# yjpark1/multiagent_rl

Measured on NVIDIA B200. Metric: agent-steps/sec, higher is better.
Workload: dtype f32

## Files before the change

multiagent_rl_b200/csrc/actor_launch.h:

```cpp
#pragma once
#include <cuda_runtime.h>
#include <stdint.h>

#include "env_launch.h"

namespace mpe {

constexpr int kActorMaxD = 64;
constexpr int kActorMaxA = 16;
constexpr int kHid = 64;
constexpr int kH = 32;
constexpr int kGateK = 96;
constexpr int kGateN = 128;

struct TcDev {
  unsigned char *blob = nullptr;
  uint32_t bytes = 0;
  int D = 0, Kx = 0, A0 = 0, A1 = 0, A = 0;
  uint32_t off_wih[2][2] = {}, off_whh[2][2] = {}, off_w1[2] = {};
  uint32_t off_w2f = 0, off_bg = 0, off_b1 = 0, off_b2 = 0;
  float *scratch = nullptr;
};

enum { kImplAuto = 0, kImplSimt = 1, kImplTc = 2, kImplTcFusedLarge = 3 };

struct ActorDev {
  TcDev tc;
  int impl = kImplAuto;
  float *blob = nullptr;
  size_t blob_floats = 0;
  size_t smem_floats = 0;
  int D = 0, A0 = 0, A1 = 0, A = 0, Apad = 0, Dpad = 0, has_model = 0;
  int off_wg[2] = {0, 0};
  int off_bg = 0;
  int off_w1 = 0;
  int off_b1 = 0;
  int off_w2 = 0;
  int off_b2 = 0;
  int off_w3 = 0;
  int off_b3 = 0;
};

struct ActorHostWeights {
  const float *dense1_w, *dense1_b, *w_ih, *w_hh, *b_ih, *b_hh, *w_ih_r, *w_hh_r, *b_ih_r, *b_hh_r;
  const float *dense2_w, *dense2_b, *dense2b_w, *dense2b_b, *dense3_w, *dense3_b;
};

struct ActorIO {
  const float *obs = nullptr;
  const float *gumbel = nullptr;
  float *logits = nullptr;
  float *next_state = nullptr;
  int32_t *act_u = nullptr, *act_c = nullptr;
  float *onehot = nullptr;
  float *hcat = nullptr;
  int64_t B = 0, gid0 = 0;
  int32_t N = 0;
  uint64_t seed = 0, step = 0;
};

struct RolloutIO {
  int32_t T = 0;
  uint64_t step0 = 0;
  float *obs_next = nullptr;
  float *rew = nullptr;
  int32_t *act_u = nullptr, *act_c = nullptr;
  float *obs_work = nullptr;
};

void actor_layout(int D, int A0, int A1, bool has_model, ActorDev *out);
void actor_pack(const ActorDev &d, const ActorHostWeights &w, float *host_blob);
bool actor_supported(int N);
bool rollout_supported(int scenario, int N);
// ... 13 lines not shown
```

multiagent_rl_b200/csrc/common.cuh:

```cuda
#pragma once
#include <cuda_runtime.h>
#include <stdint.h>

namespace mpe {

constexpr int kWarp = 32;

enum : uint32_t { kDomainReset = 1, kDomainGoal = 2, kDomainGumbel = 3, kDomainRespawn = 4 };

__device__ __forceinline__ uint4 philox4x32_10(uint4 c, uint2 k) {
#pragma unroll
  for (int r = 0; r < 10; ++r) {
    const uint32_t hi0 = __umulhi(0xD2511F53u, c.x), lo0 = 0xD2511F53u * c.x;
    const uint32_t hi1 = __umulhi(0xCD9E8D57u, c.z), lo1 = 0xCD9E8D57u * c.z;
    c = make_uint4(hi1 ^ c.y ^ k.x, lo1, hi0 ^ c.w ^ k.y, lo0);
    k.x += 0x9E3779B9u;
    k.y += 0xBB67AE85u;
  }
  return c;
}

__device__ __forceinline__ uint4 philox_raw(uint64_t seed, uint64_t gid, uint32_t t, uint32_t domain,
                                            uint32_t slot) {
  return philox4x32_10(make_uint4((uint32_t)gid, (uint32_t)(gid >> 32), t, (domain << 16) | slot),
// ... 102 lines not shown
}

__device__ __forceinline__ uint32_t smem_u32(const void *p) {
  return (uint32_t)__cvta_generic_to_shared(p);
}

__device__ __forceinline__ void fence_proxy_async_smem() {
  asm volatile("fence.proxy.async.shared::cta;" ::: "memory");
}

__device__ __forceinline__ void bulk_store(void *gdst, const void *ssrc, uint32_t bytes) {
  asm volatile("cp.async.bulk.global.shared::cta.bulk_group [%0], [%1], %2;" ::"l"(gdst),
               "r"(smem_u32(ssrc)), "r"(bytes)
               : "memory");
}
__device__ __forceinline__ void bulk_commit() { asm volatile("cp.async.bulk.commit_group;" ::: "memory"); }
__device__ __forceinline__ void bulk_wait_read_all() {
  asm volatile("cp.async.bulk.wait_group.read 0;" ::: "memory");
}
__device__ __forceinline__ void bulk_wait_read_1() {
  asm volatile("cp.async.bulk.wait_group.read 1;" ::: "memory");
}

__device__ __forceinline__ void mbar_init(uint64_t *bar, uint32_t count) {
  asm volatile("mbarrier.init.shared::cta.b64 [%0], %1;" ::"r"(smem_u32(bar)), "r"(count) : "memory");
}
__device__ __forceinline__ void mbar_fence_init() {
  asm volatile("fence.mbarrier_init.release.cluster;" ::: "memory");
}
__device__ __forceinline__ void mbar_expect_tx(uint64_t *bar, uint32_t bytes) {
  asm volatile("mbarrier.arrive.expect_tx.shared::cta.b64 _, [%0], %1;" ::"r"(smem_u32(bar)), "r"(bytes)
               : "memory");
}
__device__ __forceinline__ void mbar_wait(uint64_t *bar, uint32_t parity) {
  asm volatile(
      "{\n\t"
      ".reg .pred p;\n\t"
      "WAIT_%=:\n\t"
      "mbarrier.try_wait.parity.shared::cta.b64 p, [%0], %1, %2;\n\t"
      "@p bra DONE_%=;\n\t"
      "bra WAIT_%=;\n\t"
      "DONE_%=:\n\t"
      "}" ::"r"(smem_u32(bar)),
      "r"(parity), "r"(1000000u)
      : "memory");
}
__device__ __forceinline__ void bulk_load(void *sdst, const void *gsrc, uint32_t bytes, uint64_t *bar) {
  asm volatile(
      "cp.async.bulk.shared::cluster.global.mbarrier::complete_tx::bytes [%0], [%1], %2, [%3];" ::"r"(
          smem_u32(sdst)),
      "l"(gsrc), "r"(bytes), "r"(smem_u32(bar))
      : "memory");
}

}
```

multiagent_rl_b200/csrc/env_core.cuh:

```cuda
#pragma once
#include <cmath>
#include <type_traits>

#include "common.cuh"

namespace mpe {

enum : int { kSpread = 0, kReference = 1, kSpeaker = 2, kTreasure = 3 };

template <int SC, int N_>
struct Dims {
  static constexpr int N = N_;
  static constexpr int L = (SC == kSpread) ? N_ : 3;
  static constexpr int D = (SC == kSpread) ? 4 + 2 * L : (SC == kReference ? 21 : 11);
  static constexpr int DIMC = (SC == kSpread) ? 2 : (SC == kReference ? 10 : 3);
  static constexpr int R = N * D;
  static constexpr bool kCollide = (SC == kSpread);
  static constexpr bool kHasGoal = (SC != kSpread);
  static constexpr bool kTalks = (SC == kReference);
};

template <typename T>
struct EnvState {
  T *pv;
// ... 133 lines not shown
__device__ __forceinline__ T mul_rn(T a, T b) { return a * b; }
template <>
__device__ __forceinline__ float mul_rn<float>(float a, float b) { return __fmul_rn(a, b); }

template <typename T>
__device__ __forceinline__ void integrate_agent(T &px, T &py, T &vx, T &vy, T fx, T fy, T max_speed) {
  T vxi = mad<T>(fx, (T)0.1, mul_rn<T>(vx, (T)0.75));
  T vyi = mad<T>(fy, (T)0.1, mul_rn<T>(vy, (T)0.75));
  if (max_speed >= (T)0) {
    const T speed = sqrt(sq2<T>(vxi, vyi));
    if (speed > max_speed) {
      vxi = vxi / speed * max_speed;
      vyi = vyi / speed * max_speed;
    }
  }
  vx = vxi; vy = vyi;
  px = mad<T>(vxi, (T)0.1, px);
  py = mad<T>(vyi, (T)0.1, py);
}

template <typename T, int SC, int N>
struct Env {
  using Dm = Dims<SC, N>;
  static constexpr int L = Dm::L;
  static constexpr int D = Dm::D;
  T px[N], py[N], vx[N], vy[N];
  T lx[L], ly[L];
  int goal[2];

  __device__ __forceinline__ static T size_of_agent() {
    return SC == kSpread ? (T)0.15 : (SC == kReference ? (T)0.05 : (T)0.075);
  }
  __device__ __forceinline__ static bool movable(int i) { return !(SC == kSpeaker && i == 0); }

  __device__ __forceinline__ void load(const EnvState<T> &s, int64_t b) {
#pragma unroll
    for (int i = 0; i < N; ++i) {
      const Vec4<T> v = ld4(s.pv + ((int64_t)i * s.B + b) * 4);
      px[i] = v.x; py[i] = v.y; vx[i] = v.z; vy[i] = v.w;
    }
#pragma unroll
    for (int l = 0; l < L; ++l) {
      const Vec2<T> v = ld2(s.lm + ((int64_t)l * s.B + b) * 2);
      lx[l] = v.x; ly[l] = v.y;
    }
    goal[0] = goal[1] = -1;
    if (Dm::kHasGoal) {
      const int32_t g = s.goal[b];
      goal[0] = (g & 0xFF) == 0xFF ? -1 : (g & 0xFF);
      goal[1] = ((g >> 8) & 0xFF) == 0xFF ? -1 : ((g >> 8) & 0xFF);
    }
  }

  __device__ __forceinline__ void store_agents(const EnvState<T> &s, int64_t b) const {
#pragma unroll
    for (int i = 0; i < N; ++i) st4(s.pv + ((int64_t)i * s.B + b) * 4, Vec4<T>{px[i], py[i], vx[i], vy[i]});
  }
  __device__ __forceinline__ void store_world(const EnvState<T> &s, int64_t b) const {
#pragma unroll
    for (int l = 0; l < L; ++l) st2(s.lm + ((int64_t)l * s.B + b) * 2, Vec2<T>{lx[l], ly[l]});
    if (Dm::kHasGoal) s.goal[b] = (goal[0] & 0xFF) | ((goal[1] & 0xFF) << 8);
  }

  __device__ __forceinline__ void reset(uint64_t seed, uint64_t gid, uint32_t episode) {
    constexpr int E = N + L;
#pragma unroll
    for (int j = 0; j < (E + 1) / 2; ++j) {
      const uint4 r = philox_raw(seed, gid, episode, kDomainReset, j);
      set_entity_pos(2 * j, bits_to_pos<T>(r.x), bits_to_pos<T>(r.y));
      if (2 * j + 1 < E) set_entity_pos(2 * j + 1, bits_to_pos<T>(r.z), bits_to_pos<T>(r.w));
    }
#pragma unroll
    for (int i = 0; i < N; ++i) vx[i] = vy[i] = (T)0;
    goal[0] = goal[1] = -1;
    if (Dm::kHasGoal) {
      const uint4 r = philox_raw(seed, gid, episode, kDomainGoal, 0);
      goal[0] = (int)__umulhi(r.x, (uint32_t)L);
      if (SC == kReference) goal[1] = (int)__umulhi(r.y, (uint32_t)L);
    }
  }
  __device__ __forceinline__ void set_entity_pos(int e, T x, T y) {
    if (e < N) { px[e] = x; py[e] = y; }
    else { lx[e - N] = x; ly[e - N] = y; }
  }

  __device__ __forceinline__ void physics(const int *act_u, const EnvState<T> &s) {
    const T max_speed = s.max_speed;
    const T sens = s.accel >= (T)0 ? s.accel : (T)5.0;
    T fx[N], fy[N];
#pragma unroll
    for (int i = 0; i < N; ++i) {
      const int a = act_u[i];
      const T u0 = (T)0 + ((a == 1 ? (T)1 : (T)0) - (a == 2 ? (T)1 : (T)0));
      const T u1 = (T)0 + ((a == 3 ? (T)1 : (T)0) - (a == 4 ? (T)1 : (T)0));
      fx[i] = u0 * sens;
      fy[i] = u1 * sens;
    }
    if (Dm::kCollide) {
      const T dist_min = size_of_agent() + size_of_agent();
#pragma unroll
      for (int a = 0; a < N; ++a) {
#pragma unroll
        for (int b = a + 1; b < N; ++b) {
          const T dx = px[a] - px[b], dy = py[a] - py[b];
          const T d2 = sq2<T>(dx, dy);
          if (std::is_same<T, float>::value || !(d2 >= s.t2_cut)) {
// ... 114 lines not shown
```

multiagent_rl_b200/csrc/tc_kernels.cu:

```cuda
#include <cuda_fp16.h>

#include <cstdlib>
#include <cstring>

#include "actor_launch.h"
#include "env_core.cuh"
#include "env_group.cuh"
#include "tc_common.cuh"

namespace mpe {

constexpr int kTcThreads = 320;
constexpr int kRows = 128;
constexpr float kWScale = 16.0f, kWInv = 0.0625f, kLog2e = 1.4426950408889634f;
constexpr uint32_t kChunkA = kRows * 16;

void tc_layout(int D, int A0, int A1, TcDev *o) {
  o->D = D; o->A0 = A0; o->A1 = A1; o->A = A0 + A1;
  o->Kx = D <= 16 ? 16 : (D <= 32 ? 32 : 0);
  uint32_t off = 0;
  for (int d = 0; d < 2; ++d)
    for (int hl = 0; hl < 2; ++hl) { o->off_wih[d][hl] = off; off += kHid * kGateN * 2; }
  for (int d = 0; d < 2; ++d)
    for (int hl = 0; hl < 2; ++hl) { o->off_whh[d][hl] = off; off += kH * kGateN * 2; }
  for (int hl = 0; hl < 2; ++hl) { o->off_w1[hl] = off; off += (o->Kx > 0 ? o->Kx : 16) * kHid * 2; }
  o->off_w2f = off; off += kHid * 16 * 4;
  o->off_bg = off; off += 2 * kGateN * 4;
  o->off_b1 = off; off += kHid * 4;
  o->off_b2 = off; off += 16 * 4;
  o->bytes = (off + 127) / 128 * 128;
}

bool tc_supported(const TcDev &t) { return t.Kx > 0 && t.A <= 16; }

static void put_split(unsigned char *img, uint32_t off_hi, uint32_t off_lo, int rows, int n, int k, float v) {
  const float x = v * kWScale;
  const __half hi = __float2half_rn(x);
  const __half lo = __float2half_rn(x - __half2float(hi));
  const size_t idx = ((size_t)(k / 8) * rows + n) * 8 + (k % 8);
  reinterpret_cast<__half *>(img + off_hi)[idx] = hi;
  reinterpret_cast<__half *>(img + off_lo)[idx] = lo;
}

void tc_pack(const TcDev &t, const ActorHostWeights &w, unsigned char *img) {
  std::memset(img, 0, t.bytes);
  const float *wih[2] = {w.w_ih, w.w_ih_r}, *whh[2] = {w.w_hh, w.w_hh_r};
  const float *bih[2] = {w.b_ih, w.b_ih_r}, *bhh[2] = {w.b_hh, w.b_hh_r};
  float *bg = reinterpret_cast<float *>(img + t.off_bg);
  for (int d = 0; d < 2; ++d)
    for (int g = 0; g < 4; ++g)
      for (int u = 0; u < kH; ++u) {
        const int row = g * kH + u, n = (u >> 1) * 8 + g * 2 + (u & 1);
        for (int k = 0; k < kHid; ++k) put_split(img, t.off_wih[d][0], t.off_wih[d][1], kGateN, n, k, wih[d][row * kHid + k]);
        for (int k = 0; k < kH; ++k) put_split(img, t.off_whh[d][0], t.off_whh[d][1], kGateN, n, k, whh[d][row * kH + k]);
        bg[d * kGateN + n] = (bih[d][row] + bhh[d][row]) * (g == 2 ? -2.0f : -1.0f) * kLog2e;
      }
  float *b1 = reinterpret_cast<float *>(img + t.off_b1), *b2 = reinterpret_cast<float *>(img + t.off_b2);
  for (int j = 0; j < kHid; ++j) {
    for (int k = 0; k < t.D; ++k) put_split(img, t.off_w1[0], t.off_w1[1], kHid, j, k, w.dense1_w[j * t.D + k]);
    b1[j] = w.dense1_b[j];
  }
  for (int a = 0; a < t.A; ++a) {
    const float *src = a < t.A0 ? w.dense2_w + a * kHid : w.dense2b_w + (a - t.A0) * kHid;
    for (int k = 0; k < kHid; ++k) reinterpret_cast<float *>(img + t.off_w2f)[k * 16 + a] = src[k];
    b2[a] = a < t.A0 ? w.dense2_b[a] : w.dense2b_b[a - t.A0];
  }
}


__device__ __forceinline__ void mbar_arrive(uint64_t *bar) {
  asm volatile("mbarrier.arrive.shared::cta.b64 _, [%0];" ::"r"(smem_u32(bar)) : "memory");
}
__device__ __forceinline__ void bar_sync_n(int id, int n) { asm volatile("bar.sync %0, %1;" ::"r"(id), "r"(n) : "memory"); }

__device__ __forceinline__ void store_chunk_split(unsigned char *hi_chunk, unsigned char *lo_chunk, int row,
                                                  const float (&v)[8]) {
  uint32_t h[4], l[4];
#pragma unroll
  for (int i = 0; i < 4; ++i) {
    __half h0, l0, h1, l1;
    split_f16(v[2 * i], h0, l0);
    split_f16(v[2 * i + 1], h1, l1);
    h[i] = pack_h2(h0, h1);
    l[i] = pack_h2(l0, l1);
  }
  *reinterpret_cast<uint4 *>(hi_chunk + row * 16) = make_uint4(h[0], h[1], h[2], h[3]);
  *reinterpret_cast<uint4 *>(lo_chunk + row * 16) = make_uint4(l[0], l[1], l[2], l[3]);
}

__device__ __forceinline__ void mma3_ss(uint32_t tmem_d, const unsigned char *a_hi, const unsigned char *a_lo,
                                        uint32_t a_lbo, const unsigned char *b_hi, const unsigned char *b_lo,
                                        uint32_t b_lbo, int kblocks, uint32_t idesc, bool accumulate) {
  for (int kb = 0; kb < kblocks; ++kb) {
    const uint64_t ah = make_smem_desc(a_hi + kb * 2 * a_lbo, a_lbo, 128), al = make_smem_desc(a_lo + kb * 2 * a_lbo, a_lbo, 128);
    const uint64_t bh = make_smem_desc(b_hi + kb * 2 * b_lbo, b_lbo, 128), bl = make_smem_desc(b_lo + kb * 2 * b_lbo, b_lbo, 128);
    mma_f16_ss(tmem_d, ah, bh, idesc, accumulate || kb > 0);
    mma_f16_ss(tmem_d, al, bh, idesc, true);
    mma_f16_ss(tmem_d, ah, bl, idesc, true);
  }
}
__device__ __forceinline__ void mma3_ts(uint32_t tmem_d, uint32_t a_hi, uint32_t a_lo, const unsigned char *b_hi,
                                        const unsigned char *b_lo, uint32_t b_lbo, int kblocks, uint32_t idesc,
                                        bool accumulate) {
  for (int kb = 0; kb < kblocks; ++kb) {
    const uint64_t bh = make_smem_desc(b_hi + kb * 2 * b_lbo, b_lbo, 128), bl = make_smem_desc(b_lo + kb * 2 * b_lbo, b_lbo, 128);
    mma_f16_ts(tmem_d, a_hi + kb * 8, bh, idesc, accumulate || kb > 0);
    mma_f16_ts(tmem_d, a_lo + kb * 8, bh, idesc, true);
    mma_f16_ts(tmem_d, a_hi + kb * 8, bl, idesc, true);
  }
}

__device__ unsigned long long g_tc_timeline[148 * 128];
#ifdef MPE_TC_PHASES
#define TL(role, i)                                                                                              \
  do {                                                                                                           \
    if (dbg && first_tile && blockIdx.x < 148) g_tc_timeline[blockIdx.x * 128 + (role) * 32 + (i)] = clock64(); \
  } while (0)
#else
#define TL(role, i)
#endif

enum { B_X = 0, B_D1, B_H1, B_G, B_H, B_PER_WG };

__host__ __device__ constexpr int tc_x_slots(int N) { return N <= 3 ? N : (N <= 6 ? 4 : 2); }
__host__ __device__ inline size_t tc_x_bytes(int N, int Kx) { return (size_t)tc_x_slots(N) * 2 * (Kx / 8) * kChunkA; }
__host__ __device__ inline size_t tc_smem_bytes(uint32_t wbytes, int N, int Kx) {
  return (size_t)wbytes + 2 * (tc_x_bytes(N, Kx) + 16384 + (size_t)((kRows * N * 2 + 127) / 128 * 128)) + (1 + 2 * B_PER_WG) * 8 + 64;
}

__device__ __forceinline__ float ex2_approx(float x) {
  float y;
  asm("ex2.approx.ftz.f32 %0, %1;" : "=f"(y) : "f"(x));
  return y;
}
__device__ __forceinline__ float exp_neg(float x) { return ex2_approx(fminf(-1.4426950408889634f * x, 57.0f)); }

__device__ __forceinline__ void dense1_half(const uint32_t (&v)[32], const float *b1, uint32_t taddr_hi,
                                            uint32_t lo_off = 32) {
  uint32_t hi[16], lo[16];
#pragma unroll
  for (int j = 0; j < 16; ++j) {
    const float2 bj = *reinterpret_cast<const float2 *>(b1 + 2 * j);
    const float a0 = fmaxf(fmaf(__uint_as_float(v[2 * j]), kWInv, bj.x), 0.0f);
    const float a1 = fmaxf(fmaf(__uint_as_float(v[2 * j + 1]), kWInv, bj.y), 0.0f);
    __half h0, l0, h1, l1;
    split_f16(a0, h0, l0);
    split_f16(a1, h1, l1);
    hi[j] = pack_h2(h0, h1);
    lo[j] = pack_h2(l0, l1);
  }
  tmem_st16(taddr_hi, hi);
  tmem_st16(taddr_hi + lo_off, lo);
}

typedef unsigned long long f2;
__device__ __forceinline__ f2 pk(float lo, float hi) { f2 r; asm("mov.b64 %0, {%1, %2};" : "=l"(r) : "f"(lo), "f"(hi)); return r; }
__device__ __forceinline__ f2 pk(uint32_t lo, uint32_t hi) { f2 r; asm("mov.b64 %0, {%1, %2};" : "=l"(r) : "r"(lo), "r"(hi)); return r; }
__device__ __forceinline__ void upk(f2 v, float &lo, float &hi) { asm("mov.b64 {%0, %1}, %2;" : "=f"(lo), "=f"(hi) : "l"(v)); }
__device__ __forceinline__ f2 fma2(f2 a, f2 b, f2 c) { f2 d; asm("fma.rn.f32x2 %0, %1, %2, %3;" : "=l"(d) : "l"(a), "l"(b), "l"(c)); return d; }
__device__ __forceinline__ f2 add2(f2 a, f2 b) { f2 d; asm("add.rn.f32x2 %0, %1, %2;" : "=l"(d) : "l"(a), "l"(b)); return d; }
__device__ __forceinline__ f2 mul2(f2 a, f2 b) { f2 d; asm("mul.rn.f32x2 %0, %1, %2;" : "=l"(d) : "l"(a), "l"(b)); return d; }
__device__ __forceinline__ float rcp_approx(float x) { float y; asm("rcp.approx.ftz.f32 %0, %1;" : "=f"(y) : "f"(x)); return y; }

__device__ __forceinline__ f2 rcp2_newton(f2 d) {
  float d0, d1;
  upk(d, d0, d1);
  f2 r = pk(__uint_as_float(0x7EF311C7u - __float_as_uint(d0)), __uint_as_float(0x7EF311C7u - __float_as_uint(d1)));
  const f2 nd = mul2(d, pk(-1.0f, -1.0f)), TWO = pk(2.0f, 2.0f);
#pragma unroll
  for (int it = 0; it < 3; ++it) r = mul2(r, fma2(nd, r, TWO));
  return r;
}
// ... 430 lines not shown
          if (mine) {
            if (do_reset) {
              const uint32_t ep = s.episode[b] + 1u;
              s.episode[b] = ep;
              e.reset(s.seed, (uint64_t)(s.gid0 + b), ep);
              e.store_world(s, b);
              if (SC == kReference) {
#pragma unroll
                for (int i = 0; i < 2; ++i)
#pragma unroll
                  for (int k = 0; k < 10; ++k) comm[i][k] = 0.0f;
              }
            }
            e.store_agents(s, b);
            if (SC == kReference) {
#pragma unroll
              for (int i = 0; i < 2; ++i)
#pragma unroll
                for (int k = 0; k < 10; ++k) s.comm[((int64_t)i * 10 + k) * s.B + b] = comm[i][k];
            }
          }
          if (row == 0 && tma_ok && (g_obs != nullptr || g_rew != nullptr)) bulk_wait_read_all();
        } else {
          bar_sync_n(1 + g, 128);
          const int rows = valid * N;
          if (io.act_u != nullptr)
            for (int i = row; i < rows; i += 128) io.act_u[env0 * N + i] = sm_act[i * 2];
          if (io.act_c != nullptr)
            for (int i = row; i < rows; i += 128) io.act_c[env0 * N + i] = sm_act[i * 2 + 1];
          if (io.onehot != nullptr)
            for (int i = row; i < rows * w.A; i += 128) {
              const int rr = i / w.A, a = i - rr * w.A;
              const bool hot = a < w.A0 ? (a == sm_act[rr * 2]) : (a - w.A0 == sm_act[rr * 2 + 1]);
              io.onehot[env0 * N * w.A + i] = hot ? 1.0f : 0.0f;
            }
        }
        TL(g, 29);
        bar_sync_n(1 + g, 128);
        TL(g, 30);
      }
    }
  }
  tc_fence_before();
  __syncthreads();
  if (warp == 8) tmem_free(tmem_base, 512);
}

#endif

__host__ __device__ inline size_t tc2_tile_bytes(int N, int Kx, int APAD) {
  return tc_x_bytes(N, Kx) + 16384 + (size_t)((kRows * N * 2 + 127) / 128 * 128) + (N <= 3 && APAD <= 8 ? (size_t)N * APAD * kRows * 4 : 0);
}
enum { B2_XR = 0, B2_XF = 4, B2_OBS = 8, B2_EXTRA = 9 };
__host__ __device__ inline size_t tc2_smem_bytes(uint32_t wbytes, int N, int Kx, int APAD) {
  return (size_t)wbytes + 2 * tc2_tile_bytes(N, Kx, APAD) + (1 + 2 * B_PER_WG + 2 * B2_EXTRA) * 8 + 64;
}
__host__ __device__ inline size_t tc2_scratch_f2_per_cta(int N, int APAD) { return (size_t)2 * 2 * 2 * N * (APAD / 2) * kRows; }
__host__ __device__ constexpr int tc2_threads(int N) { return N > 3 ? 384 : 320; }

template <int SC, int N, bool FUSED, int APAD>
__global__ void __launch_bounds__(tc2_threads(N), 1)
    k_tc2(EnvState<float> s, TcDev w, ActorIO io, RolloutIO ro, int max_episode_len, int64_t ntiles, int dbg) {
  constexpr bool kJit = N > 3;
  constexpr bool kXs = !kJit && APAD > 8;
  static_assert(!(kJit && FUSED) || (SC == kSpread && group_lanes(N) > 0), "fused large-team rollout: simple_spread, 6..12 agents");
  extern __shared__ __align__(128) unsigned char smem[];
#ifdef MPE_TC_PHASES
  if (dbg && threadIdx.x == 0 && blockIdx.x < 148) {
    unsigned long long gt;
    asm volatile("mov.u64 %0, %%globaltimer;" : "=l"(gt));
    g_tc_timeline[blockIdx.x * 128 + 64] = gt;
    g_tc_timeline[blockIdx.x * 128 + 66] = clock64();
  }
#endif
  using Dm = Dims<SC, N>;
  const int D = FUSED ? Dm::D : w.D;
  const int R = N * D;
  const int Kx = w.Kx;
  const int tid = threadIdx.x, warp = tid >> 5;
  const size_t xb = tc_x_bytes(N, Kx);
  const size_t tile_bytes = tc2_tile_bytes(N, Kx, APAD);
  unsigned char *sm_w = smem;
  uint64_t *bars = reinterpret_cast<uint64_t *>(smem + w.bytes + 2 * tile_bytes);
  uint64_t *xbars = bars + 1 + 2 * B_PER_WG;
  uint32_t *tmem_slot = reinterpret_cast<uint32_t *>(xbars + 2 * B2_EXTRA);
  auto tile_smem = [&](int X) { return smem + w.bytes + X * tile_bytes; };

  if (tid == 0) {
    mbar_init(&bars[0], 1);
    for (int g = 0; g < 2; ++g) {
      uint64_t *bb = bars + 1 + g * B_PER_WG;
      mbar_init(&bb[B_X], 128);
      mbar_init(&bb[B_D1], 1);
      mbar_init(&bb[B_H1], 256);
      mbar_init(&bb[B_G], 1);
      mbar_init(&bb[B_H], 256);
      for (int q = 0; q < 4; ++q) {
        mbar_init(&xbars[g * B2_EXTRA + B2_XR + q], 32);
        mbar_init(&xbars[g * B2_EXTRA + B2_XF + q], 1);
      }
      mbar_init(&xbars[g * B2_EXTRA + B2_OBS], 128);
    }
    mbar_fence_init();
    mbar_expect_tx(&bars[0], w.bytes);
    bulk_load(sm_w, w.blob, w.bytes, &bars[0]);
  }
  if (warp == 8) tmem_alloc(tmem_slot, 512);
  tc_fence_before();
  __syncthreads();
  tc_fence_after();
  const uint32_t tmem_base = *tmem_slot;
  const int T = FUSED ? ro.T : 1;
  auto agent_of = [](int k) { return k < N ? k : 2 * N - 1 - k; };
  auto need_e1 = [&](int k) { return k < N || agent_of(k) + 2 < N; };
  auto slot_col = [](int t) { return 128u + 64u * (uint32_t)(t & 1); };
  const int64_t npairs = (ntiles + 1) / 2;
  auto d1_index = [](int j) { return j < N ? j : j - 2; };
  constexpr int kRing = kJit ? tc_x_slots(N) : 1;

  if (kJit && warp >= 10) {
    const int X = warp - 10, lane = tid & 31;
    unsigned char *sm_x = tile_smem(X);
    uint64_t *xb2 = xbars + X * B2_EXTRA;
    uint32_t ph_xf = 0, filled = 0, ph_obs = 0;
    const float *obs_src = FUSED ? ro.obs_work : io.obs;
    const int64_t nbx = FUSED ? s.B : io.B;
    const bool vec2 = (reinterpret_cast<uintptr_t>(obs_src) & 7) == 0 && (D & 1) == 0;
    for (int64_t pair = blockIdx.x; pair < npairs; pair += gridDim.x) {
      const int64_t tile = pair * 2 + X, env0 = tile * kRows;
      const int valid = tile < ntiles ? (int)((nbx - env0) < kRows ? (nbx - env0) : kRows) : 0;
#pragma unroll 1
      for (int it = 0; it < T; ++it) {
        if (FUSED && it > 0) {
          mbar_wait(&xb2[B2_OBS], ph_obs);
          ph_obs ^= 1;
        }
#pragma unroll 1
        for (int j = 0; j < 2 * N; ++j) {
          if (!need_e1(j)) continue;
          const int t = agent_of(j), q = d1_index(j) & (kRing - 1);
          if ((filled >> q) & 1u) { mbar_wait(&xb2[B2_XF + q], (ph_xf >> q) & 1u); ph_xf ^= 1u << q; }
          filled |= 1u << q;
          unsigned char *xh = sm_x + (size_t)(q * 2) * (Kx / 8) * kChunkA, *xl = xh + (size_t)(Kx / 8) * kChunkA;
#pragma unroll 1
          for (int rp = 0; rp < 2; ++rp) {
            float xr[2][32];
#pragma unroll
            for (int u = 0; u < 2; ++u) {
              const int r = lane + 32 * (2 * rp + u);
#pragma unroll
              for (int k = 0; k < 32; ++k) xr[u][k] = 0.0f;
              if (r < valid) {
                const float *src = obs_src + (env0 + r) * R + t * D;
                if (vec2) {
#pragma unroll
                  for (int k = 0; k < 16; ++k)
                    if (2 * k < D) {
                      const float2 v = *reinterpret_cast<const float2 *>(src + 2 * k);
                      xr[u][2 * k] = v.x; xr[u][2 * k + 1] = v.y;
                    }
                } else {
#pragma unroll
                  for (int k = 0; k < 32; ++k)
                    if (k < D) xr[u][k] = src[k];
                }
              }
            }
#pragma unroll
            for (int u = 0; u < 2; ++u) {
              const int r = lane + 32 * (2 * rp + u);
#pragma unroll
              for (int c = 0; c < 4; ++c) {
                if (c * 8 < Kx) {
                  const float v[8] = {xr[u][c * 8], xr[u][c * 8 + 1], xr[u][c * 8 + 2], xr[u][c * 8 + 3],
                                      xr[u][c * 8 + 4], xr[u][c * 8 + 5], xr[u][c * 8 + 6], xr[u][c * 8 + 7]};
                  store_chunk_split(xh + c * kChunkA, xl + c * kChunkA, r, v);
                }
              }
            }
          }
          fence_proxy_async_smem();
          mbar_arrive(&xb2[B2_XR + q]);
        }
      }
    }
  } else if (warp >= 8) {
    const int X = warp - 8;
    if ((tid & 31) == 0) {
      unsigned char *sm_x = tile_smem(X), *sm_h = sm_x + xb;
      uint64_t *bb = bars + 1 + X * B_PER_WG;
      const uint32_t tmem = tmem_base + X * 256;
      uint32_t ph_x = 0, ph_h1 = 0, ph_h = 0, ph_xr = 0;
      uint64_t *xb2 = xbars + X * B2_EXTRA;
      const uint32_t id_g = make_idesc_f16(128, 128), id_d1 = make_idesc_f16(128, 64);
      mbar_wait(&bars[0], 0);
      for (int64_t pair = blockIdx.x; pair < npairs; pair += gridDim.x) {
        for (int it = 0; it < T; ++it) {
          if constexpr (!kJit) {
            mbar_wait(&bb[B_X], ph_x); ph_x ^= 1;
            tc_fence_after();
          }
          auto dense1_cell = [&](int j) {
            const int t = agent_of(j), q = d1_index(j) & (kRing - 1), xs = kJit ? q : t;
            if constexpr (kJit) {
              mbar_wait(&xb2[B2_XR + q], (ph_xr >> q) & 1u); ph_xr ^= 1u << q;
              tc_fence_after();
            }
            const unsigned char *xh = sm_x + (size_t)(xs * 2) * (Kx / 8) * kChunkA, *xl = xh + (size_t)(Kx / 8) * kChunkA;
            mma3_ss(tmem + slot_col(t), xh, xl, kChunkA, sm_w + w.off_w1[0], sm_w + w.off_w1[1], kHid * 16, Kx / 16, id_d1, false);
            mma_commit(&bb[B_D1]);
            if constexpr (kJit) mma_commit(&xb2[B2_XF + q]);
          };
          dense1_cell(0);
          for (int k = 0; k < 2 * N; ++k) {
            const int d = k >= N ? 1 : 0, st = k - d * N;
            if (need_e1(k)) { mbar_wait(&bb[B_H1], ph_h1); ph_h1 ^= 1; }
            if (k > 0) { mbar_wait(&bb[B_H], ph_h); ph_h ^= 1; }
            tc_fence_after();
            const uint32_t a0 = tmem + slot_col(agent_of(k));
            const unsigned char *wih_hi = sm_w + (d ? w.off_wih[1][0] : w.off_wih[0][0]);
            const unsigned char *wih_lo = sm_w + (d ? w.off_wih[1][1] : w.off_wih[0][1]);
            mma3_ts(tmem, a0, a0 + 16, wih_hi, wih_lo, kGateN * 16, 2, id_g, false);
            mma3_ts(tmem, a0 + 32, a0 + 48, wih_hi + 4 * kGateN * 16, wih_lo + 4 * kGateN * 16, kGateN * 16, 2, id_g, true);
            if (st > 0) mma3_ss(tmem, sm_h, sm_h + 8192, kChunkA, sm_w + (d ? w.off_whh[1][0] : w.off_whh[0][0]),
                                sm_w + (d ? w.off_whh[1][1] : w.off_whh[0][1]), kGateN * 16, 2, id_g, true);
            mma_commit(&bb[B_G]);
            if (k + 1 < 2 * N && need_e1(k + 1)) dense1_cell(k + 1);
          }
          mbar_wait(&bb[B_H], ph_h); ph_h ^= 1;
        }
      }
    }
    __syncwarp();
  } else {
    const int half = tid >> 7, own = half, row = tid & 127;
    const uint32_t lane_base = (uint32_t)(row & ~31) << 16;
    const float *b1 = reinterpret_cast<const float *>(sm_w + w.off_b1);
    const float *b2 = reinterpret_cast<const float *>(sm_w + w.off_b2);
    const float *w2f = reinterpret_cast<const float *>(sm_w + w.off_w2f);
    unsigned char *own_x = tile_smem(own), *own_h = own_x + xb;
    uint8_t *own_act = own_h + 16384;
    [[maybe_unused]] const f2 *own_xchg2 = reinterpret_cast<const f2 *>(own_act + (kRows * N * 2 + 127) / 128 * 128);
    float *stage_obs = reinterpret_cast<float *>(own_x), *stage_rew = stage_obs + kRows * R;
    uint32_t ph_d1[2] = {0, 0}, ph_g[2] = {0, 0};
    bool tma_pending = false;
    f2 *scr = (kJit || kXs) ? reinterpret_cast<f2 *>(w.scratch) + (size_t)blockIdx.x * tc2_scratch_f2_per_cta(N, APAD) : nullptr;
    bool have_w = false;
#ifdef MPE_TC_PHASES
    if (dbg && tid == 0 && blockIdx.x < 148) g_tc_timeline[blockIdx.x * 128 + 67] = clock64();
#endif
    for (int64_t pair = blockIdx.x; pair < npairs; pair += gridDim.x) {
#ifdef MPE_TC_PHASES
      if (dbg && tid == 0 && blockIdx.x < 148 && pair != blockIdx.x) g_tc_timeline[blockIdx.x * 128 + 68] = clock64();
#endif
      const int64_t tile = pair * 2 + own;
      const int64_t env0 = tile * kRows;
      const int64_t nb = FUSED ? s.B : io.B;
      const int valid = tile < ntiles ? (int)((nb - env0) < kRows ? (nb - env0) : kRows) : 0;
      const bool mine = row < valid;
      const int64_t b = env0 + row;
      [[maybe_unused]] const bool first_tile = pair == blockIdx.x && row == 0;
      for (int it = 0; it < T; ++it) {
        TL(half, 0);
        if constexpr (!kJit) {
          Env<float, SC, N> e;
          float comm[2][10];
          if (FUSED && mine) {
            e.load(s, b);
            if (SC == kReference) {
#pragma unroll
              for (int i = 0; i < 2; ++i)
#pragma unroll
                for (int k = 0; k < 10; ++k) comm[i][k] = s.comm[((int64_t)i * 10 + k) * s.B + b];
            }
          }
          if (FUSED) {
            if (tma_pending) bulk_wait_read_all();
            tma_pending = false;
            bar_sync_n(2 + own, 128);
          }
#pragma unroll
          for (int t = 0; t < N; ++t) {
            float xr[32];
#pragma unroll
            for (int k = 0; k < 32; ++k) xr[k] = 0.0f;
            if (FUSED) {
              if (mine) e.obs_row(t, xr, SC == kReference ? comm[1 - (t & 1)] : nullptr);
            } else if (mine) {
              const float *src = io.obs + b * R + t * D;
#pragma unroll
              for (int k = 0; k < 32; ++k)
                if (k < D) xr[k] = src[k];
            }
            unsigned char *xh = own_x + (size_t)(t * 2) * (Kx / 8) * kChunkA, *xl = xh + (size_t)(Kx / 8) * kChunkA;
#pragma unroll
            for (int c = 0; c < 4; ++c) {
              if (c * 8 < Kx) {
                const float v[8] = {xr[c * 8], xr[c * 8 + 1], xr[c * 8 + 2], xr[c * 8 + 3],
                                    xr[c * 8 + 4], xr[c * 8 + 5], xr[c * 8 + 6], xr[c * 8 + 7]};
                store_chunk_split(xh + c * kChunkA, xl + c * kChunkA, row, v);
              }
            }
          }
        }
        if constexpr (!kJit) {
          fence_proxy_async_smem();
          mbar_arrive(&bars[1 + own * B_PER_WG + B_X]);
        }

        if (!have_w) { mbar_wait(&bars[0], 0); have_w = true; }
        constexpr int NLG = kJit ? 1 : N;
        f2 lgp[NLG][APAD / 2];
#pragma unroll
        for (int t = 0; t < NLG; ++t)
#pragma unroll
          for (int a = 0; a < APAD / 2; ++a) lgp[t][a] = pk(b2[2 * a], b2[2 * a + 1]);

        f2 cA[2][4], cB[2][4];
#ifdef MPE_TC_PHASES
        uint32_t acc[10] = {0, 0, 0, 0, 0, 0, 0, 0, 0, 0}, tlast = clock();
#define TS(i)                                   \
  do {                                          \
    if (dbg) {                                  \
      const uint32_t now = clock();             \
      acc[i] += now - tlast;                    \
      tlast = now;                              \
    }                                           \
  } while (0)
#else
#define TS(i)
#endif
        auto E1 = [&](auto XT, int k) {
          constexpr int X = decltype(XT)::value;
          uint64_t *bb = bars + 1 + X * B_PER_WG;
          const uint32_t tmem = tmem_base + X * 256 + slot_col(agent_of(k)) + half * 32;
          TS(9);
          mbar_wait(&bb[B_D1], ph_d1[X]); ph_d1[X] ^= 1;
          tc_fence_after();
          TS(0);
          uint32_t v0[32];
          tmem_ld32(tmem + lane_base, v0);
          tmem_wait_ld();
          TS(1);
          dense1_half(v0, b1 + half * 32, tmem + lane_base, 16);
          TS(2);
          tmem_wait_st();
          tc_fence_before();
          mbar_arrive(&bb[B_H1]);
          TS(3);
        };
        auto CC = [&](auto XT, int k, f2 (&c)[2][4]) {
          constexpr int X = decltype(XT)::value;
          const int d = k >= N ? 1 : 0, st = k - d * N;
          [[maybe_unused]] const int t = d == 0 ? st : N - 1 - st;
          uint64_t *bb = bars + 1 + X * B_PER_WG;
          const uint32_t tmem = tmem_base + X * 256;
          unsigned char *sm_h = tile_smem(X) + xb;
          if (st == 0) {
#pragma unroll
            for (int q = 0; q < 4; ++q) c[0][q] = c[1][q] = 0ull;
          }
          const float *bg = reinterpret_cast<const float *>(sm_w + w.off_bg) + d * kGateN + half * 64;
          const float *w2d = w2f + (d * kH + half * 16) * 16;
          f2 pl[APAD / 2];
#pragma unroll
          for (int a = 0; a < APAD / 2; ++a) pl[a] = 0ull;
          TS(9);
          mbar_wait(&bb[B_G], ph_g[X]); ph_g[X] ^= 1;
          tc_fence_after();
          TS(4);
          {
            float *hc = nullptr;
            if constexpr (!FUSED) {
              if (io.hcat != nullptr) {
                const int64_t bx = (pair * 2 + X) * (int64_t)kRows + row;
                if (bx < io.B) hc = io.hcat + (bx * N + (d == 0 ? st : N - 1 - st)) * kHid + d * kH + half * 16;
              }
            }
            uint32_t va[32], vb[32];
            tmem_ld32(tmem + lane_base + half * 64, va);
            tmem_wait_ld();
            TS(5);
            tmem_ld32(tmem + lane_base + half * 64 + 32, vb);
            lstm_chunk<APAD>(va, bg, w2d, c[0], pl, sm_h + (2 * half) * kChunkA, row, st < N - 1, hc);
            TS(6);
            tmem_wait_ld();
            TS(7);
            lstm_chunk<APAD>(vb, bg + 32, w2d + 8 * 16, c[1], pl, sm_h + (2 * half + 1) * kChunkA, row, st < N - 1,
                             hc != nullptr ? hc + 8 : nullptr);
          }
          fence_proxy_async_smem();
          tc_fence_before();
          mbar_arrive(&bb[B_H]);
          TS(8);
          if constexpr (kJit) {
            f2 *dst = scr + ((size_t)((X * 2 + half) * 2 * N + k) * (APAD / 2)) * kRows + row;
#pragma unroll
            for (int a = 0; a < APAD / 2; ++a) dst[a * kRows] = pl[a];
          } else if (X == own) {
#pragma unroll
            for (int tt = 0; tt < NLG; ++tt)
              if (tt == t) {
#pragma unroll
                for (int a = 0; a < APAD / 2; ++a) lgp[tt][a] = add2(lgp[tt][a], pl[a]);
              }
          } else if constexpr (kXs) {
            f2 *dst = scr + ((size_t)((X * 2 + half) * 2 * N + k) * (APAD / 2)) * kRows + row;
#pragma unroll
// ... 333 lines not shown
                bulk_commit();
              }
            } else {
              if (g_obs != nullptr)
                for (int i = row; i < valid * R; i += 128) g_obs[i] = stage_obs[i];
              if (g_rew != nullptr)
                for (int i = row; i < valid * N; i += 128) g_rew[i] = stage_rew[i];
            }
          }
          if (ro.act_u != nullptr)
            for (int i = row; i < valid * N; i += 128) ro.act_u[(toff + env0) * N + i] = own_act[i * 2];
          if (ro.act_c != nullptr)
            for (int i = row; i < valid * N; i += 128) ro.act_c[(toff + env0) * N + i] = own_act[i * 2 + 1];
          if (mine) {
            if (do_reset) {
              const uint32_t ep = s.episode[b] + 1u;
              s.episode[b] = ep;
              e.reset(s.seed, (uint64_t)(s.gid0 + b), ep);
              e.store_world(s, b);
              if (SC == kReference) {
#pragma unroll
                for (int i = 0; i < 2; ++i)
#pragma unroll
                  for (int k = 0; k < 10; ++k) comm[i][k] = 0.0f;
              }
            }
            e.store_agents(s, b);
            if (SC == kReference) {
#pragma unroll
              for (int i = 0; i < 2; ++i)
#pragma unroll
                for (int k = 0; k < 10; ++k) s.comm[((int64_t)i * 10 + k) * s.B + b] = comm[i][k];
            }
          }
          TL(half, 23);
          if (row == 0 && tma_ok && (g_obs != nullptr || g_rew != nullptr)) tma_pending = true;
        } else {
          bar_sync_n(2 + own, 128);
          const int rows = valid * N;
          if (io.act_u != nullptr)
            for (int i = row; i < rows; i += 128) io.act_u[env0 * N + i] = own_act[i * 2];
          if (io.act_c != nullptr)
            for (int i = row; i < rows; i += 128) io.act_c[env0 * N + i] = own_act[i * 2 + 1];
          if (io.onehot != nullptr)
            for (int i = row; i < rows * w.A; i += 128) {
              const int rr = i / w.A, a = i - rr * w.A;
              const bool hot = a < w.A0 ? (a == own_act[rr * 2]) : (a - w.A0 == own_act[rr * 2 + 1]);
              io.onehot[env0 * N * w.A + i] = hot ? 1.0f : 0.0f;
            }
        }
        TL(half, 30);
        bar_sync_n(1, 256);
        TL(half, 31);
      }
    }
    if (tma_pending) bulk_wait_read_all();
  }
  tc_fence_before();
  __syncthreads();
  if (warp == 8) tmem_free(tmem_base, 512);
#ifdef MPE_TC_PHASES
  if (dbg && threadIdx.x == 0 && blockIdx.x < 148) {
    unsigned long long gt;
    asm volatile("mov.u64 %0, %%globaltimer;" : "=l"(gt));
    g_tc_timeline[blockIdx.x * 128 + 65] = gt;
    g_tc_timeline[blockIdx.x * 128 + 69] = clock64();
  }
#endif
}

static int current_device() {
  int dev = 0;
  cudaGetDevice(&dev);
  return (dev >= 0 && dev < 64) ? dev : 0;
}
static int sm_count_tc(int dev) {
  static int cached[64] = {0};
  if (cached[dev] == 0) {
    int n = 0;
    cudaDeviceGetAttribute(&n, cudaDevAttrMultiProcessorCount, dev);
    cached[dev] = n > 0 ? n : 148;
  }
  return cached[dev];
}
template <typename K>
static cudaError_t ensure_smem(K kernel, size_t bytes, size_t (&have)[64], int dev) {
  if (have[dev] >= bytes) return cudaSuccess;
  cudaError_t e = cudaFuncSetAttribute(kernel, cudaFuncAttributeMaxDynamicSharedMemorySize, (int)bytes);
  if (e == cudaSuccess) have[dev] = bytes;
  return e;
}
static int tc_debug_flag() {
  static const int dbg = getenv("MPE_TC_TIMELINE") != nullptr ? 1 : 0;
  return dbg;
}

template <int SC, int N, bool FUSED, int APAD>
static cudaError_t launch_tc2_t(const EnvState<float> &s, const TcDev &w, const ActorIO &io, const RolloutIO &ro,
                                int max_episode_len, int64_t nenvs, cudaStream_t st) {
  static size_t have[64] = {0};
  const int dev = current_device();
  const size_t smem = tc2_smem_bytes(w.bytes, N, w.Kx, APAD);
  cudaError_t e = ensure_smem(k_tc2<SC, N, FUSED, APAD>, smem, have, dev);
  if (e != cudaSuccess) return e;
  const int64_t ntiles = (nenvs + kRows - 1) / kRows;
  const int nsm = sm_count_tc(dev);
  const int64_t pairs = (ntiles + 1) / 2;
  const int grid = (int)(pairs < nsm ? pairs : nsm);
// ... 32 lines not shown
}
size_t tc_scratch_floats(int sm_count) {
#ifdef MPE_AB_KERNELS
  const size_t v1 = (size_t)sm_count * 2 * 12 * 16 * kRows;
#else
  const size_t v1 = 0;
#endif
  const size_t v2 = (size_t)sm_count * tc2_scratch_f2_per_cta(12, 8) * 2, v3 = (size_t)sm_count * tc2_scratch_f2_per_cta(3, 16) * 2;
  return v1 > v2 ? (v1 > v3 ? v1 : v3) : (v2 > v3 ? v2 : v3);
}

cudaError_t launch_actor_forward_tc(const TcDev &w, const ActorIO &io, cudaStream_t st) {
  EnvState<float> s{};
  RolloutIO ro;
  const bool wide = w.A > 8;
  switch (io.N) {
    case 2: return wide ? launch_tc_t<kSpread, 2, false, 16>(s, w, io, ro, 0, io.B, st)
                        : launch_tc_t<kSpread, 2, false, 8>(s, w, io, ro, 0, io.B, st);
    case 3: return wide ? launch_tc_t<kSpread, 3, false, 16>(s, w, io, ro, 0, io.B, st)
                        : launch_tc_t<kSpread, 3, false, 8>(s, w, io, ro, 0, io.B, st);
    case 4: return wide ? cudaErrorInvalidValue : launch_tc_t<kSpread, 4, false, 8>(s, w, io, ro, 0, io.B, st);
    case 6: return wide ? cudaErrorInvalidValue : launch_tc_t<kSpread, 6, false, 8>(s, w, io, ro, 0, io.B, st);
    case 8: return wide ? cudaErrorInvalidValue : launch_tc_t<kSpread, 8, false, 8>(s, w, io, ro, 0, io.B, st);
    case 9: return wide ? cudaErrorInvalidValue : launch_tc_t<kSpread, 9, false, 8>(s, w, io, ro, 0, io.B, st);
    case 12: return wide ? cudaErrorInvalidValue : launch_tc_t<kSpread, 12, false, 8>(s, w, io, ro, 0, io.B, st);
    default: return cudaErrorInvalidValue;
  }
}

cudaError_t launch_rollout_tc(const EnvStateAny &a, const TcDev &w, const RolloutIO &ro, cudaStream_t st) {
  EnvState<float> s;
  s.pv = static_cast<float *>(a.pv); s.lm = static_cast<float *>(a.lm); s.goal = a.goal; s.episode = a.episode;
  s.tstep = a.tstep; s.ep_ret = static_cast<float *>(a.ep_ret); s.comm = static_cast<float *>(a.comm);
  s.stats = a.stats; s.B = a.B; s.gid0 = a.gid0; s.seed = a.seed; s.max_speed = (float)a.max_speed;
  s.accel = (float)a.accel; s.track = 1;
  set_thresholds<float>(s, a.scenario);
  ActorIO io;
  if (a.scenario == kReference) return launch_tc_t<kReference, 2, true, 16>(s, w, io, ro, a.max_episode_len, a.B, st);
  if (a.scenario == kSpeaker) return launch_tc_t<kSpeaker, 2, true, 8>(s, w, io, ro, a.max_episode_len, a.B, st);
  if (a.N == 2) return launch_tc_t<kSpread, 2, true, 8>(s, w, io, ro, a.max_episode_len, a.B, st);
  if (a.N == 3) return launch_tc_t<kSpread, 3, true, 8>(s, w, io, ro, a.max_episode_len, a.B, st);
  if (ro.obs_work == nullptr) return cudaErrorInvalidValue;
  if (a.N == 6) return launch_tc_t<kSpread, 6, true, 8>(s, w, io, ro, a.max_episode_len, a.B, st);
  if (a.N == 9) return launch_tc_t<kSpread, 9, true, 8>(s, w, io, ro, a.max_episode_len, a.B, st);
  if (a.N == 12) return launch_tc_t<kSpread, 12, true, 8>(s, w, io, ro, a.max_episode_len, a.B, st);
  return cudaErrorInvalidValue;
}

}

extern "C" __attribute__((visibility("default"))) int mpe_debug_tc_timeline(unsigned long long *out, int n) {
  return (int)cudaMemcpyFromSymbol(out, mpe::g_tc_timeline, sizeof(unsigned long long) * (size_t)n);
}
```

Baseline: 3.046 billion.

## Split weight TMA load into pieces and prefetch env state into L1/L2

```diff
diff --git a/multiagent_rl_b200/csrc/actor_launch.h b/multiagent_rl_b200/csrc/actor_launch.h
--- a/multiagent_rl_b200/csrc/actor_launch.h
+++ b/multiagent_rl_b200/csrc/actor_launch.h
@@ -19,6 +19,7 @@
   int D = 0, Kx = 0, A0 = 0, A1 = 0, A = 0;
   uint32_t off_wih[2][2] = {}, off_whh[2][2] = {}, off_w1[2] = {};
   uint32_t off_w2f = 0, off_bg = 0, off_b1 = 0, off_b2 = 0;
+  uint32_t piece_end[3] = {};
   float *scratch = nullptr;
 };
 
diff --git a/multiagent_rl_b200/csrc/common.cuh b/multiagent_rl_b200/csrc/common.cuh
--- a/multiagent_rl_b200/csrc/common.cuh
+++ b/multiagent_rl_b200/csrc/common.cuh
@@ -178,5 +178,9 @@
       "l"(gsrc), "r"(bytes), "r"(smem_u32(bar))
       : "memory");
 }
+__device__ __forceinline__ void prefetch_l1(const void *p) { asm volatile("prefetch.global.L1 [%0];" ::"l"(p)); }
+__device__ __forceinline__ void prefetch_l2_bulk(const void *p, uint32_t bytes) {
+  asm volatile("cp.async.bulk.prefetch.L2.global [%0], %1;" ::"l"(p), "r"(bytes) : "memory");
+}
 
 }
diff --git a/multiagent_rl_b200/csrc/env_core.cuh b/multiagent_rl_b200/csrc/env_core.cuh
--- a/multiagent_rl_b200/csrc/env_core.cuh
+++ b/multiagent_rl_b200/csrc/env_core.cuh
@@ -209,6 +209,21 @@
     }
   }
 
+  __device__ __forceinline__ static void prefetch(const EnvState<T> &s, int64_t b) {
+#pragma unroll
+    for (int i = 0; i < N; ++i) prefetch_l1(s.pv + ((int64_t)i * s.B + b) * 4);
+#pragma unroll
+    for (int l = 0; l < L; ++l) prefetch_l1(s.lm + ((int64_t)l * s.B + b) * 2);
+    if (Dm::kHasGoal) prefetch_l1(s.goal + b);
+  }
+  __device__ __forceinline__ static void prefetch_l2(const EnvState<T> &s, int64_t e0, int n) {
+#pragma unroll
+    for (int i = 0; i < N; ++i) prefetch_l2_bulk(s.pv + ((int64_t)i * s.B + e0) * 4, (uint32_t)(n * 4 * sizeof(T)));
+#pragma unroll
+    for (int l = 0; l < L; ++l) prefetch_l2_bulk(s.lm + ((int64_t)l * s.B + e0) * 2, (uint32_t)(n * 2 * sizeof(T)));
+    if (Dm::kHasGoal) prefetch_l2_bulk(s.goal + e0, (uint32_t)(n * 4));
+  }
+
   __device__ __forceinline__ void store_agents(const EnvState<T> &s, int64_t b) const {
 #pragma unroll
     for (int i = 0; i < N; ++i) st4(s.pv + ((int64_t)i * s.B + b) * 4, Vec4<T>{px[i], py[i], vx[i], vy[i]});
diff --git a/multiagent_rl_b200/csrc/tc_kernels.cu b/multiagent_rl_b200/csrc/tc_kernels.cu
--- a/multiagent_rl_b200/csrc/tc_kernels.cu
+++ b/multiagent_rl_b200/csrc/tc_kernels.cu
@@ -19,16 +19,19 @@
   o->D = D; o->A0 = A0; o->A1 = A1; o->A = A0 + A1;
   o->Kx = D <= 16 ? 16 : (D <= 32 ? 32 : 0);
   uint32_t off = 0;
-  for (int d = 0; d < 2; ++d)
-    for (int hl = 0; hl < 2; ++hl) { o->off_wih[d][hl] = off; off += kHid * kGateN * 2; }
-  for (int d = 0; d < 2; ++d)
-    for (int hl = 0; hl < 2; ++hl) { o->off_whh[d][hl] = off; off += kH * kGateN * 2; }
   for (int hl = 0; hl < 2; ++hl) { o->off_w1[hl] = off; off += (o->Kx > 0 ? o->Kx : 16) * kHid * 2; }
   o->off_w2f = off; off += kHid * 16 * 4;
   o->off_bg = off; off += 2 * kGateN * 4;
   o->off_b1 = off; off += kHid * 4;
   o->off_b2 = off; off += 16 * 4;
-  o->bytes = (off + 127) / 128 * 128;
+  off = (off + 127) / 128 * 128;
+  o->piece_end[0] = off;
+  for (int d = 0; d < 2; ++d) {
+    for (int hl = 0; hl < 2; ++hl) { o->off_wih[d][hl] = off; off += kHid * kGateN * 2; }
+    for (int hl = 0; hl < 2; ++hl) { o->off_whh[d][hl] = off; off += kH * kGateN * 2; }
+    o->piece_end[1 + d] = off;
+  }
+  o->bytes = off;
 }
 
 bool tc_supported(const TcDev &t) { return t.Kx > 0 && t.A <= 16; }
@@ -116,8 +119,13 @@
   do {                                                                                                           \
     if (dbg && first_tile && blockIdx.x < 148) g_tc_timeline[blockIdx.x * 128 + (role) * 32 + (i)] = clock64(); \
   } while (0)
+#define TC_STAMP(slot)                                                                      \
+  do {                                                                                      \
+    if (dbg && blockIdx.x < 148) g_tc_timeline[blockIdx.x * 128 + (slot)] = clock64();      \
+  } while (0)
 #else
 #define TL(role, i)
+#define TC_STAMP(slot) do {} while (0)
 #endif
 
 enum { B_X = 0, B_D1, B_H1, B_G, B_H, B_PER_WG };
@@ -654,8 +662,9 @@
   return tc_x_bytes(N, Kx) + 16384 + (size_t)((kRows * N * 2 + 127) / 128 * 128) + (N <= 3 && APAD <= 8 ? (size_t)N * APAD * kRows * 4 : 0);
 }
 enum { B2_XR = 0, B2_XF = 4, B2_OBS = 8, B2_EXTRA = 9 };
+constexpr int kWBars = 3;
 __host__ __device__ inline size_t tc2_smem_bytes(uint32_t wbytes, int N, int Kx, int APAD) {
-  return (size_t)wbytes + 2 * tc2_tile_bytes(N, Kx, APAD) + (1 + 2 * B_PER_WG + 2 * B2_EXTRA) * 8 + 64;
+  return (size_t)wbytes + 2 * tc2_tile_bytes(N, Kx, APAD) + (kWBars + 2 * B_PER_WG + 2 * B2_EXTRA) * 8 + 64;
 }
 __host__ __device__ inline size_t tc2_scratch_f2_per_cta(int N, int APAD) { return (size_t)2 * 2 * 2 * N * (APAD / 2) * kRows; }
 __host__ __device__ constexpr int tc2_threads(int N) { return N > 3 ? 384 : 320; }
@@ -684,14 +693,34 @@
   const size_t tile_bytes = tc2_tile_bytes(N, Kx, APAD);
   unsigned char *sm_w = smem;
   uint64_t *bars = reinterpret_cast<uint64_t *>(smem + w.bytes + 2 * tile_bytes);
-  uint64_t *xbars = bars + 1 + 2 * B_PER_WG;
+  uint64_t *xbars = bars + kWBars + 2 * B_PER_WG;
   uint32_t *tmem_slot = reinterpret_cast<uint32_t *>(xbars + 2 * B2_EXTRA);
   auto tile_smem = [&](int X) { return smem + w.bytes + X * tile_bytes; };
 
+  if constexpr (FUSED && !kJit) {
+    const int64_t b = ((int64_t)blockIdx.x * 2 + (tid >> 7)) * kRows + (tid & 127);
+    if (warp < 8 && b < s.B) {
+      Env<float, SC, N>::prefetch(s, b);
+      if (SC == kReference) {
+#pragma unroll
+        for (int i = 0; i < 20; ++i) prefetch_l1(s.comm + (int64_t)i * s.B + b);
+      }
+    }
+  }
+  if (warp == 9 && (tid & 31) == 0) {
+#pragma unroll
+    for (int p = 0; p < kWBars; ++p) mbar_init(&bars[p], 1);
+    mbar_fence_init();
+#pragma unroll
+    for (int p = 0; p < kWBars; ++p) {
+      const uint32_t lo = p > 0 ? w.piece_end[p - 1] : 0u, len = w.piece_end[p] - lo;
+      mbar_expect_tx(&bars[p], len);
+      bulk_load(sm_w + lo, w.blob + lo, len, &bars[p]);
+    }
+  }
   if (tid == 0) {
-    mbar_init(&bars[0], 1);
     for (int g = 0; g < 2; ++g) {
-      uint64_t *bb = bars + 1 + g * B_PER_WG;
+      uint64_t *bb = bars + kWBars + g * B_PER_WG;
       mbar_init(&bb[B_X], 128);
       mbar_init(&bb[B_D1], 1);
       mbar_init(&bb[B_H1], 256);
@@ -704,8 +733,6 @@
       mbar_init(&xbars[g * B2_EXTRA + B2_OBS], 128);
     }
     mbar_fence_init();
-    mbar_expect_tx(&bars[0], w.bytes);
-    bulk_load(sm_w, w.blob, w.bytes, &bars[0]);
   }
   if (warp == 8) tmem_alloc(tmem_slot, 512);
   tc_fence_before();
@@ -790,14 +817,29 @@
     const int X = warp - 8;
     if ((tid & 31) == 0) {
       unsigned char *sm_x = tile_smem(X), *sm_h = sm_x + xb;
-      uint64_t *bb = bars + 1 + X * B_PER_WG;
+      uint64_t *bb = bars + kWBars + X * B_PER_WG;
       const uint32_t tmem = tmem_base + X * 256;
       uint32_t ph_x = 0, ph_h1 = 0, ph_h = 0, ph_xr = 0;
       uint64_t *xb2 = xbars + X * B2_EXTRA;
       const uint32_t id_g = make_idesc_f16(128, 128), id_d1 = make_idesc_f16(128, 64);
       mbar_wait(&bars[0], 0);
+      if (X == 0) TC_STAMP(70);
       for (int64_t pair = blockIdx.x; pair < npairs; pair += gridDim.x) {
+        if constexpr (FUSED && !kJit) {
+          const int64_t e0 = (pair + gridDim.x) * 2 * kRows;
+          const int n = (int)((s.B - e0 < 2 * kRows ? s.B - e0 : 2 * kRows) & ~3);
+          const bool aligned = ((s.B & 3) == 0) && ((reinterpret_cast<uintptr_t>(s.pv) | reinterpret_cast<uintptr_t>(s.lm) |
+                                                     reinterpret_cast<uintptr_t>(s.goal) | reinterpret_cast<uintptr_t>(s.comm)) & 15) == 0;
+          if (X == 1 && n > 0 && aligned) {
+            Env<float, SC, N>::prefetch_l2(s, e0, n);
+            if (SC == kReference) {
+#pragma unroll 1
+              for (int i = 0; i < 20; ++i) prefetch_l2_bulk(s.comm + (int64_t)i * s.B + e0, (uint32_t)n * 4);
+            }
+          }
+        }
         for (int it = 0; it < T; ++it) {
+          [[maybe_unused]] const bool first_step = X == 0 && pair == blockIdx.x && it == 0;
           if constexpr (!kJit) {
             mbar_wait(&bb[B_X], ph_x); ph_x ^= 1;
             tc_fence_after();
@@ -814,10 +856,12 @@
             if constexpr (kJit) mma_commit(&xb2[B2_XF + q]);
           };
           dense1_cell(0);
+          if (first_step) TC_STAMP(72);
           for (int k = 0; k < 2 * N; ++k) {
             const int d = k >= N ? 1 : 0, st = k - d * N;
             if (need_e1(k)) { mbar_wait(&bb[B_H1], ph_h1); ph_h1 ^= 1; }
             if (k > 0) { mbar_wait(&bb[B_H], ph_h); ph_h ^= 1; }
+            if (st == 0) mbar_wait(&bars[1 + d], 0);
             tc_fence_after();
             const uint32_t a0 = tmem + slot_col(agent_of(k));
             const unsigned char *wih_hi = sm_w + (d ? w.off_wih[1][0] : w.off_wih[0][0]);
@@ -827,6 +871,7 @@
             if (st > 0) mma3_ss(tmem, sm_h, sm_h + 8192, kChunkA, sm_w + (d ? w.off_whh[1][0] : w.off_whh[0][0]),
                                 sm_w + (d ? w.off_whh[1][1] : w.off_whh[0][1]), kGateN * 16, 2, id_g, true);
             mma_commit(&bb[B_G]);
+            if (first_step && k == 0) TC_STAMP(73);
             if (k + 1 < 2 * N && need_e1(k + 1)) dense1_cell(k + 1);
           }
           mbar_wait(&bb[B_H], ph_h); ph_h ^= 1;
@@ -907,8 +952,9 @@
         }
         if constexpr (!kJit) {
           fence_proxy_async_smem();
-          mbar_arrive(&bars[1 + own * B_PER_WG + B_X]);
+          mbar_arrive(&bars[kWBars + own * B_PER_WG + B_X]);
         }
+        if (tid == 0 && pair == blockIdx.x && it == 0) TC_STAMP(71);
 
         if (!have_w) { mbar_wait(&bars[0], 0); have_w = true; }
         constexpr int NLG = kJit ? 1 : N;
@@ -934,7 +980,7 @@
 #endif
         auto E1 = [&](auto XT, int k) {
           constexpr int X = decltype(XT)::value;
-          uint64_t *bb = bars + 1 + X * B_PER_WG;
+          uint64_t *bb = bars + kWBars + X * B_PER_WG;
           const uint32_t tmem = tmem_base + X * 256 + slot_col(agent_of(k)) + half * 32;
           TS(9);
           mbar_wait(&bb[B_D1], ph_d1[X]); ph_d1[X] ^= 1;
@@ -955,7 +1001,7 @@
           constexpr int X = decltype(XT)::value;
           const int d = k >= N ? 1 : 0, st = k - d * N;
           [[maybe_unused]] const int t = d == 0 ? st : N - 1 - st;
-          uint64_t *bb = bars + 1 + X * B_PER_WG;
+          uint64_t *bb = bars + kWBars + X * B_PER_WG;
           const uint32_t tmem = tmem_base + X * 256;
           unsigned char *sm_h = tile_smem(X) + xb;
           if (st == 0) {
@@ -1395,8 +1441,10 @@
         TL(half, 30);
         bar_sync_n(1, 256);
         TL(half, 31);
+        if (tid == 0 && pair == blockIdx.x && it == 0) TC_STAMP(75);
       }
     }
+    if (tid == 0) TC_STAMP(74);
     if (tma_pending) bulk_wait_read_all();
   }
   tc_fence_before();
@@ -1535,3 +1583,19 @@
 extern "C" __attribute__((visibility("default"))) int mpe_debug_tc_timeline(unsigned long long *out, int n) {
   return (int)cudaMemcpyFromSymbol(out, mpe::g_tc_timeline, sizeof(unsigned long long) * (size_t)n);
 }
+
+#ifdef MPE_TC_PHASES
+__device__ unsigned long long g_tc_marks[8];
+__global__ void k_tc_mark(int slot) {
+  unsigned long long gt;
+  asm volatile("mov.u64 %0, %%globaltimer;" : "=l"(gt));
+  g_tc_marks[slot] = gt;
+}
+extern "C" __attribute__((visibility("default"))) int mpe_debug_tc_mark(int slot, void *stream) {
+  k_tc_mark<<<1, 1, 0, static_cast<cudaStream_t>(stream)>>>(slot & 7);
+  return (int)cudaGetLastError();
+}
+extern "C" __attribute__((visibility("default"))) int mpe_debug_tc_marks(unsigned long long *out) {
+  return (int)cudaMemcpyFromSymbol(out, g_tc_marks, sizeof(g_tc_marks));
+}
+#endif
```

Measured after the change: 3.108 billion, median of 6. +2.0%, better.
